# zhiqiangdon/pose-adv-aug

Measured on AMD Instinct MI355X. Metric: images/sec, 2-stack HG 256x256 bs=24 per GPU, full training step, higher is better.
Workload: dtype bf16; 1 GPU; BASELINE configs[1]: 2-stack hourglass chan 256, bs=24/GPU, 256x256 MPII-shape synthetic frames (720x1280 uint8 resident in HBM), on-device HumanAug warp, heat-map MSE, RMSprop, PCKh; global_batch=24, parallelism=dp1, ranks_seen=1, devices_seen=1

## Files before the change

pose_adv_aug_amd/csrc/api.hip:

```cpp
#include "../../include/poseadv.h"
#include "net.h"
#include "warp_bwd.h"
#include <stdio.h>
#include <string.h>
#include <new>
#include <string>

static thread_local char g_err[1024] = "";
void pa_set_error(const char* what, hipError_t e, const char* file, int line) {
    snprintf(g_err, sizeof g_err, "%s:%d: %s -> %s", file, line, what, hipGetErrorString(e));
}
void pa_set_error_msg(const char* msg) { snprintf(g_err, sizeof g_err, "%s", msg); }

struct pa_net { Net n; };
#define ST(s) reinterpret_cast<hipStream_t>(s)
#define TRY(x) do { int _r = (x); if (_r) { if (!g_err[0]) pa_set_error("kernel launch", (hipError_t)_r, __FILE__, __LINE__); return _r; } } while (0)
#define NEED_PTR(fn, p) do { if (!(p)) { pa_set_error_msg(fn ": " #p " is NULL"); return 1; } } while (0)
#define NEED_POS(fn, v) do { if ((v) < 1) { pa_set_error_msg(fn ": " #v " must be >= 1"); return 1; } } while (0)

extern "C" {

const char* pa_last_error(void) { return g_err; }
float pa_grad_scale(void) { return PA_GRAD_SCALE; }
int pa_dtype(void) { return PA_DTYPE_ID; }
// ... 321 lines not shown
    float* pbuf = nullptr; float* gbuf = nullptr;
    PA_CHECK(hipMallocAsync((void**)&pbuf, n.n_params * sizeof(float) * 2 + 64, n.st));
    gbuf = pbuf + ((n.n_params + 3) & ~(size_t)3);
    PA_CHECK(hipMemsetAsync(pbuf, 0, n.n_params * sizeof(float) * 2 + 64, n.st));
    PA_CHECK(hipMemcpyAsync(pbuf + op.c.p_w, w, (size_t)Cout * Cin * k * k * sizeof(float), hipMemcpyDeviceToDevice, n.st));
    if (bias) PA_CHECK(hipMemcpyAsync(pbuf + op.c.p_b, bias, Cout * sizeof(float), hipMemcpyDeviceToDevice, n.st));
    n.params = pbuf; n.grads = gbuf; n.buffers = pbuf;
    TRY(n.upload_tables());
    TRY(n.prepare_weights());
    n.train_bn = false;
    if (mode == 0) {
        TRY(pa_launch_nchw_f32_to_nhwc_bf16(a_in, op.xin, B, Cin, H, W, n.st));
        TRY(n.conv_fwd(op.c, pa_plain(op.xin), B, H, W, pa_none(), pa_none(), op.yout, nullptr));
        TRY(pa_launch_nhwc_bf16_to_nchw_f32(pa_plain(op.yout), out, B, Cout, H, W, n.st));
    } else if (mode == 1) {
        PaEpilogue ep; memset(&ep, 0, sizeof ep); ep.mode = PA_OUT_PLAIN;
        TRY(pa_launch_nchw_f32_to_nhwc_bf16(a_in, op.yout, B, Cout, H, W, n.st));
        TRY(n.conv_dgrad(op.c, pa_plain(op.yout), B, H, W, pa_none(), pa_none(), ep, op.xin));
        TRY(pa_launch_nhwc_bf16_to_nchw_f32(pa_plain(op.xin), out, B, Cin, H, W, n.st));
    } else {
        TRY(pa_launch_nchw_f32_to_nhwc_bf16(a_in, op.yout, B, Cout, H, W, n.st));
        TRY(pa_launch_nchw_f32_to_nhwc_bf16(b_in, op.xin, B, Cin, H, W, n.st));
        TRY(n.conv_wgrad(op.c, pa_plain(op.yout), pa_plain(op.xin), B, H, W));
        TRY(n.reduce_grads());
        PA_CHECK(hipMemcpyAsync(out, gbuf + op.c.p_w, (size_t)Cout * Cin * k * k * sizeof(float), hipMemcpyDeviceToDevice, n.st));
        if (out2) PA_CHECK(hipMemcpyAsync(out2, gbuf + op.c.p_b, Cout * sizeof(float), hipMemcpyDeviceToDevice, n.st));
    }
    PA_CHECK(hipStreamSynchronize(n.st));
    PA_CHECK(hipFree(pbuf));
    return 0;
}

struct WgradGroupOp {
    Net n; ConvLayer c[PA_WG_GROUP_MAX]; bf16 *dy[PA_WG_GROUP_MAX], *dyq[PA_WG_GROUP_MAX], *x[PA_WG_GROUP_MAX];
    float *pbuf = nullptr, *gbuf = nullptr;
    size_t build(const pa_wgrad_job* jobs, int nj, char* base) {
        Arena a; a.base = base;
        n.prep_jobs = a.get<PaPrepJob>(nj); n.red_jobs = a.get<PaWgradReduceJob>(nj); n.bneval_jobs = a.get<PaBnEvalJob>(1);
        for (int j = 0; j < nj; ++j) {
            const pa_wgrad_job& q = jobs[j];
            n.B = q.B;
            n.layout_conv(c[j], a, q.B * q.H * q.W, q.H, q.W);
            const size_t M = (size_t)q.B * q.H * q.W;
            dy[j] = a.get<bf16>(M * c[j].pcout);
            dyq[j] = q.dy_q ? a.get<bf16>(M * c[j].pcout) : nullptr;
            x[j] = a.get<bf16>(M * c[j].pcin);
        }
        pbuf = a.get<float>(n.n_params + 8);
        gbuf = a.get<float>(n.n_params + 8);
        a.take(0);
        return a.off;
    }
    int declare(const pa_wgrad_job* jobs, int nj) {
        if (nj < 1 || nj > PA_WG_GROUP_MAX) { pa_set_error_msg("pa_wgrad_group: 1 .. 8 jobs"); return 1; }
        n.is_agent = true;
        for (int j = 0; j < nj; ++j) {
            const pa_wgrad_job& q = jobs[j];
            if (q.Cin % 64 || q.Cout % 64 || (q.k != 1 && q.k != 3) || q.B < 1 || q.H < 1 || q.W < 1) { pa_set_error_msg("pa_wgrad_group: channels % 64 == 0, k in {1,3}"); return 1; }
            if ((q.dy_q == nullptr) != (q.dy_k == nullptr)) { pa_set_error_msg("pa_wgrad_group: dy_q and dy_k come together"); return 1; }
            char name[16]; snprintf(name, sizeof name, "j%d", j);
            n.declare_conv(c[j], name, q.Cin, q.Cout, q.k, q.db == nullptr);
        }
        return 0;
    }
};

size_t pa_wgrad_group_workspace_bytes(const pa_wgrad_job* jobs, int njobs) {
    g_err[0] = 0;
    WgradGroupOp op;
    if (op.declare(jobs, njobs)) return 0;
    return op.build(jobs, njobs, nullptr);
}

int pa_wgrad_group(const pa_wgrad_job* jobs, int njobs, int mode, void* ws, void* s) {
    g_err[0] = 0;
    WgradGroupOp op; Net& n = op.n;
    TRY(op.declare(jobs, njobs));
    n.st = ST(s);
    op.build(jobs, njobs, reinterpret_cast<char*>(ws));
    PA_CHECK(hipMemsetAsync(op.gbuf, 0, (n.n_params + 8) * sizeof(float), n.st));
    n.params = op.pbuf; n.grads = op.gbuf; n.buffers = op.pbuf;
    TRY(n.upload_tables());
    PaWgradArgs args[PA_WG_GROUP_MAX]; const PaWgradArgs* ptrs[PA_WG_GROUP_MAX];
    for (int j = 0; j < njobs; ++j) {
        const pa_wgrad_job& q = jobs[j];
        ConvLayer& c = op.c[j];
        TRY(pa_launch_nchw_f32_to_nhwc_bf16(q.dy, op.dy[j], q.B, q.Cout, q.H, q.W, n.st));
        if (q.dy_q) TRY(pa_launch_nchw_f32_to_nhwc_bf16(q.dy_q, op.dyq[j], q.B, q.Cout, q.H, q.W, n.st));
        TRY(pa_launch_nchw_f32_to_nhwc_bf16(q.x, op.x[j], q.B, q.Cin, q.H, q.W, n.st));
        PaWgradArgs& a = args[j]; memset(&a, 0, sizeof a);
        a.dy = pa_plain(op.dy[j]);
        if (q.dy_q) { a.dy.mode = PA_LD_LIN2; a.dy.q = op.dyq[j]; a.dy.k0 = q.dy_k; a.dy.k1 = q.dy_k + q.Cout; a.dy.k2 = q.dy_k + 2 * q.Cout; }
        a.x = pa_plain(op.x[j]);
        if (q.x_k) { a.x.mode = PA_LD_BNRELU; a.x.k0 = q.x_k; a.x.k1 = q.x_k + q.Cin; }
        a.part = c.part; a.dbpart = c.dbpart;
        a.B = q.B; a.H = q.H; a.W = q.W; a.Cin = c.pcin; a.Cout = c.pcout; a.taps = c.taps(); a.splits = c.splits;
        ptrs[j] = &a;
    }
    if (mode == 0) {
        for (int j = 0; j < njobs; ++j) TRY(pa_launch_wgrad(args[j], n.st));
    } else {
        for (int j = 0; j < njobs; ++j)
            if (pa_wgrad_job_workgroups(args[j]) == 0) { pa_set_error_msg("pa_wgrad_group: a job the grouped kernel does not take (shape / operand modes)"); return 2; }
        TRY(pa_launch_wgrad_group(ptrs, njobs, n.st, mode == 2));
    }
    TRY(pa_launch_wgrad_reduce(n.red_jobs, n.n_red, n.red_max, n.st));
    for (int j = 0; j < njobs; ++j) {
        const pa_wgrad_job& q = jobs[j];
        PA_CHECK(hipMemcpyAsync(q.dw, op.gbuf + op.c[j].p_w, (size_t)q.Cout * q.Cin * q.k * q.k * sizeof(float), hipMemcpyDeviceToDevice, n.st));
        if (q.db) PA_CHECK(hipMemcpyAsync(q.db, op.gbuf + op.c[j].p_b, q.Cout * sizeof(float), hipMemcpyDeviceToDevice, n.st));
    }
    PA_CHECK(hipStreamSynchronize(n.st));
    return 0;
}

int pa_conv2d_time(int mode, int variant, int B, int Cin, int Cout, int H, int W, int k, int iters, void* ws, float* ms_out, void* s) {
    g_err[0] = 0;
    ConvOp op; Net& n = op.n; n.is_agent = true; n.B = B; n.st = ST(s);
    n.declare_conv(op.c, "c", Cin, Cout, k, false);
    BNLayer bn_in, bn_out;
    n.declare_bn(bn_in, "bi", mode == 0 ? Cin : Cout);
    n.declare_bn(bn_out, "bo", mode == 0 ? Cout : Cin);
    Arena a; a.base = reinterpret_cast<char*>(ws);
    a.off = op.build(B, H, W, a.base);
    for (BNLayer* b : n.bns) n.layout_bn(*b, a, B * H * W);
    const size_t M = (size_t)B * H * W;
    bf16* extra = a.get<bf16>(M * (Cin > Cout ? Cin : Cout));
    bf16* extra2 = a.get<bf16>(M * (Cin > Cout ? Cin : Cout));
    float* pbuf = a.get<float>(2 * (n.n_params + 8));
    n.params = pbuf; n.grads = pbuf + n.n_params + 8; n.buffers = pbuf;
// ... 537 lines not shown
```

pose_adv_aug_amd/csrc/conv_wgrad.hip:

```cpp
#include "common.h"
#include "kernels.h"
#include "wgrad_reduce.h"
#include <stdlib.h>

template <int TN, int TK, int PMODE, int QMODE, int TAPS, bool STEM = false>
__global__ __launch_bounds__(256) void conv_wgrad_kernel(PaWgradArgs a) {
    constexpr int NI = TN / 32, KI = TK / 32;
    constexpr int MS = (TN + TK <= 128) ? 128 : 64;
    constexpr int MG = MS / 8;
    constexpr int NP = MG * TN / 8, NQ = MG * TK / 8;
    __shared__ __attribute__((aligned(16))) bf16 lds[(TN + TK) * MS];
    bf16* Pt = lds;
    bf16* Qt = lds + TN * MS;

    const int tid = threadIdx.x, lane = tid & 63, wave = tid >> 6;
    const int wn = wave & 1, wk = wave >> 1;
    const int M = a.B * a.H * a.W, HW = a.H * a.W;
    const int Kfull = TAPS * a.Cin;
    const int ktiles_per_tap = a.Cin / TK;
    const int split = blockIdx.x;
    const int tap = blockIdx.y / ktiles_per_tap;
    const int cbase = (blockIdx.y - tap * ktiles_per_tap) * TK;
    const int nbase = blockIdx.z * TN;
    const int dy = (TAPS == 9) ? tap / 3 - 1 : 0, dx = (TAPS == 9) ? tap - (tap / 3) * 3 - 1 : 0;
// ... 175 lines not shown
            float s = colsum[c];
            s += __shfl_xor(s, 1, 64); s += __shfl_xor(s, 2, 64); s += __shfl_xor(s, 4, 64);
            if (MG == 16) s += __shfl_xor(s, 8, 64);
            if (mg == 0) a.dbpart[(size_t)split * a.Cout + chan + c] = s;
        }
    }
}

template <int TN, int TK, int PMODE, int QMODE>
static void launch_w_taps(const PaWgradArgs& a, dim3 grid, hipStream_t st) {
    if (a.taps == 1) hipLaunchKernelGGL((conv_wgrad_kernel<TN, TK, PMODE, QMODE, 1>), grid, dim3(256), 0, st, a);
    else hipLaunchKernelGGL((conv_wgrad_kernel<TN, TK, PMODE, QMODE, 9>), grid, dim3(256), 0, st, a);
}

template <int TN, int TK>
static void launch_w_modes(const PaWgradArgs& a, dim3 grid, hipStream_t st) {
    const bool lin2 = a.dy.mode == PA_LD_LIN2, bnrelu = a.x.mode == PA_LD_BNRELU;
    if (lin2 && bnrelu) launch_w_taps<TN, TK, PA_LD_LIN2, PA_LD_BNRELU>(a, grid, st);
    else if (lin2) launch_w_taps<TN, TK, PA_LD_LIN2, PA_LD_PLAIN>(a, grid, st);
    else if (bnrelu) launch_w_taps<TN, TK, PA_LD_PLAIN, PA_LD_BNRELU>(a, grid, st);
    else launch_w_taps<TN, TK, PA_LD_PLAIN, PA_LD_PLAIN>(a, grid, st);
}

int pa_launch_stem_wgrad(const PaWgradArgs& a, hipStream_t st) {
    if (a.Cin != 256 || a.Cout != 64 || a.taps != 1 || a.x.mode != PA_LD_PLAIN || a.splits < 1) {
        pa_set_error_msg("pa_launch_stem_wgrad: bad arguments");
        return 1;
    }
    const PaWgradPlan p = pa_wgrad_launch_plan(a.B, a.H, a.W, a.Cin, a.Cout, a.taps, true, a.splits, false);
    if (p.path == PA_WGP_STEM_TILE) return pa_launch_stem_wgrad_tile(a, p, st);
    dim3 grid(a.splits, p.blocks, 1);
    if (a.dy.mode == PA_LD_LIN2)
        hipLaunchKernelGGL((conv_wgrad_kernel<64, 128, PA_LD_LIN2, PA_LD_PLAIN, 1, true>), grid, dim3(256), 0, st, a);
    else
        hipLaunchKernelGGL((conv_wgrad_kernel<64, 128, PA_LD_PLAIN, PA_LD_PLAIN, 1, true>), grid, dim3(256), 0, st, a);
    return (int)hipGetLastError();
}

int pa_launch_wgrad(const PaWgradArgs& a, hipStream_t st) {
    if ((a.taps != 1 && a.taps != 9) || a.Cin % 64 != 0 || a.Cout % 64 != 0 || a.splits < 1) {
        pa_set_error_msg("pa_launch_wgrad: channel counts must be multiples of 64, taps 1 or 9, splits >= 1");
        return 1;
    }
    const PaWgradPlan p = pa_wgrad_launch_plan(a.B, a.H, a.W, a.Cin, a.Cout, a.taps, false, a.splits, a.dbpart != nullptr);
    if (p.path == PA_WGP_TILE) return pa_launch_wgrad_tile(a, p, st);
    dim3 grid(a.splits, a.taps * a.Cin / p.cb, a.Cout / p.nb);
    if (p.nb == 128 && p.cb == 128) launch_w_modes<128, 128>(a, grid, st);
    else if (p.nb == 128) launch_w_modes<128, 64>(a, grid, st);
    else if (p.cb == 128) launch_w_modes<64, 128>(a, grid, st);
    else launch_w_modes<64, 64>(a, grid, st);
    return (int)hipGetLastError();
}

__global__ void wgrad_reduce_kernel(const PaWgradReduceJob* jobs) {
    wgrad_reduce_body(jobs[blockIdx.y], (int)blockIdx.x, (int)gridDim.x);
}

__global__ void wgrad_reduce_list_kernel(const PaWgradReduceJob* jobs, PaRedList list) {
    wgrad_reduce_body(jobs[list.idx[blockIdx.y]], (int)blockIdx.x, (int)gridDim.x);
}

int pa_launch_wgrad_reduce_list(const PaWgradReduceJob* jobs_dev, const int* idx, int n, int max_elems, hipStream_t st) {
    if (n <= 0) return 0;
    if (n > PA_RED_LIST_MAX) { pa_set_error_msg("pa_launch_wgrad_reduce_list: too many jobs"); return 1; }
    PaRedList list;
    for (int i = 0; i < PA_RED_LIST_MAX; ++i) list.idx[i] = idx[i < n ? i : 0];
    int bx = (max_elems + 255) / 256;
    if (bx > 576) bx = 576;
    if (bx < 1) bx = 1;
    hipLaunchKernelGGL(wgrad_reduce_list_kernel, dim3(bx, n), dim3(256), 0, st, jobs_dev, list);
    return (int)hipGetLastError();
}

int pa_launch_wgrad_reduce(const PaWgradReduceJob* jobs_dev, int njobs, int max_elems, hipStream_t st) {
    if (njobs <= 0) return 0;
    int bx = (max_elems + 255) / 256;
    if (bx > 576) bx = 576;
    if (bx < 1) bx = 1;
    hipLaunchKernelGGL(wgrad_reduce_kernel, dim3(bx, njobs), dim3(256), 0, st, jobs_dev);
    return (int)hipGetLastError();
}

__global__ __launch_bounds__(1024) void stem_wgrad_reduce_kernel(const float* part, int splits, float* dst, float* zero64) {
    __shared__ float red[4][256];
    const int n = blockIdx.x, k = threadIdx.x & 255, sl = threadIdx.x >> 8;
    if (zero64 && n == 0 && threadIdx.x < 64) zero64[threadIdx.x] = 0.f;
    const float* src = part + (size_t)n * 256 + k;
    float s = 0.f;
#pragma unroll 8
    for (int sp = sl; sp < splits; sp += 4) s += src[(size_t)sp * 64 * 256];
    red[sl][k] = s;
    __syncthreads();
    if (sl == 0) {
        const int ky = k >> 5, kx = (k & 31) >> 2, c = k & 3;
        if (ky < 7 && kx < 7 && c < 3) dst[((size_t)(n * 3 + c) * 7 + ky) * 7 + kx] = red[0][k] + red[1][k] + red[2][k] + red[3][k];
    }
}

int pa_launch_stem_wgrad_reduce(const float* part, int splits, float* dst, hipStream_t st, float* zero64) {
    hipLaunchKernelGGL(stem_wgrad_reduce_kernel, dim3(64), dim3(1024), 0, st, part, splits, dst, zero64);
    return (int)hipGetLastError();
}
```

pose_adv_aug_amd/csrc/conv_wgrad_tile.hip:

```cpp
#include "common.h"
#include "kernels.h"
#include "wgrad_reduce.h"
#include <stdlib.h>
#include <string.h>
#include <hip/hip_ext.h>

#ifndef PA_WG_NT
#define PA_WG_NT 0
#endif
#if PA_WG_NT
#define PA_WG_LOAD(p) __builtin_nontemporal_load(p)
#define PA_WG_STORE(p, v) __builtin_nontemporal_store(v, p)
#else
#define PA_WG_LOAD(p) (*(p))
#define PA_WG_STORE(p, v) (*(p) = (v))
#endif
#define PA_WG_RT 7
#define PA_WG_STEM 3
typedef short s16x4 __attribute__((ext_vector_type(4)));
typedef short s16x8 __attribute__((ext_vector_type(8)));

template <int CH>
__device__ __forceinline__ int wg_sw(int p) {
    return CH >= 128 ? ((p & 3) | ((p >> 1) & 4)) : (((p >> 1) & 1) | ((p >> 2) & 2));
}

template <int CH, class PixFn>
__device__ __forceinline__ bf16x8 wg_tr_frag(const bf16* tile, int gran, PixFn pix) {
    const int l = threadIdx.x & 63;
    s16x4 h[2];
#pragma unroll
    for (int hh = 0; hh < 2; ++hh) {
        const int p = pix(8 * (l >> 4) + 4 * hh + ((l & 15) >> 2));
        const bf16* ptr = tile + p * CH + ((gran ^ wg_sw<CH>(p)) << 4) + 4 * (l & 3);
        h[hh] = __builtin_amdgcn_ds_read_tr16_b64_v4i16((__attribute__((address_space(3))) s16x4*)(ptr));
    }
    s16x8 v = __builtin_shufflevector(h[0], h[1], 0, 1, 2, 3, 4, 5, 6, 7);
    return __builtin_bit_cast(bf16x8, v);
}

__device__ __forceinline__ void wg_lds_barrier() { asm volatile("s_waitcnt lgkmcnt(0)\n\ts_barrier" ::: "memory"); }

template <int TAPS, int NF, int CF, int WNW>
constexpr int wg_lds_elems() { return 128 * (16 * NF * WNW) + (TAPS == 9 ? 10 * 32 : 128) * (16 * CF * (4 / WNW)); }

template <int TAPS, int NF, int CF, int WNW, int PMODE, int QMODE, bool DB, bool PIPE>
__device__ __forceinline__ void wgrad_tile_body(const PaWgradArgs& a, int ntiles, int split, int S, int by, int bz, bf16* lds) {
    constexpr int WCW = 4 / WNW;
    constexpr int NB = 16 * NF * WNW, CB = 16 * CF * WCW;
    constexpr int PW = 18, PWL = 32, HP = TAPS == 9 ? 180 : 128, HPL = TAPS == 9 ? 10 * PWL : 128;
    constexpr int CPN = NB / 8, CPC = CB / 8;
    constexpr int PASS_N = 128 * CPN / 256;
    constexpr int PASS_C = (HP * CPC + 255) / 256;
    static_assert(128 * NB + HPL * CB == wg_lds_elems<TAPS, NF, CF, WNW>(), "LDS size");
    bf16* dyT = lds;
    bf16* xT = lds + 128 * NB;

    const int tid = threadIdx.x, lane = tid & 63;
    const int wave = __builtin_amdgcn_readfirstlane(tid >> 6);
    const int wn = wave % WNW, wc = wave / WNW;
    const int n0 = by * NB, c0 = bz * CB;
    const int M = a.B * a.H * a.W;
    const int tiles_x = TAPS == 9 ? a.W / 16 : 1, tiles_y = TAPS == 9 ? a.H / 8 : 1;
    const int Kfull = TAPS * a.Cin;

    const int nchunk = tid % CPN, cchunk = tid % CPC;
    const bool want_db = DB && a.dbpart != nullptr && bz == 0;
    const bool p_lin2 = PMODE == PA_LD_LIN2 || (PMODE == PA_WG_RT && a.dy.mode == PA_LD_LIN2);
    const bool q_bnrelu = QMODE == PA_LD_BNRELU || (QMODE == PA_WG_RT && a.x.mode == PA_LD_BNRELU);
    static_assert(!PIPE || (PMODE != PA_WG_RT && QMODE != PA_WG_RT), "run-time modes: plain form only");
    float colsum[8];
#pragma unroll
    for (int j = 0; j < 8; ++j) colsum[j] = 0.f;

    f32x4 acc[TAPS][CF][NF];
#pragma unroll
    for (int t = 0; t < TAPS; ++t)
#pragma unroll
        for (int cf = 0; cf < CF; ++cf)
#pragma unroll
            for (int f = 0; f < NF; ++f) acc[t][cf][f] = f32x4{0.f, 0.f, 0.f, 0.f};

    auto mfma_tile = [&]() {
        if (TAPS == 9) {
            int doff[NF][2], xoff[3][2];
#pragma unroll
            for (int hh = 0; hh < 2; ++hh) {
                const int kl = 8 * (lane >> 4) + 4 * hh + ((lane & 15) >> 2);
#pragma unroll
                for (int f = 0; f < NF; ++f) doff[f][hh] = kl * NB + (((wn * NF + f) ^ wg_sw<NB>(kl)) << 4) + 4 * (lane & 3);
#pragma unroll
                for (int d = 0; d < 3; ++d) {
                    const int col = (kl & 15) + d;
                    xoff[d][hh] = ((kl >> 4) * PWL + col) * CB + ((wc ^ wg_sw<CB>(col)) << 4) + 4 * (lane & 3);
                }
            }
            auto tr8 = [&](const bf16* base, int o0, int o1) {
                s16x4 h0 = __builtin_amdgcn_ds_read_tr16_b64_v4i16((__attribute__((address_space(3))) s16x4*)(base + o0));
                s16x4 h1 = __builtin_amdgcn_ds_read_tr16_b64_v4i16((__attribute__((address_space(3))) s16x4*)(base + o1));
                s16x8 v = __builtin_shufflevector(h0, h1, 0, 1, 2, 3, 4, 5, 6, 7);
// ... 165 lines not shown
            __builtin_amdgcn_sched_barrier(0);
            wg_lds_barrier();
            mfma_tile();
        }
    } else
    for (int tile = split; tile < ntiles; tile += S) {
        int b = 0, y0 = 0, x0 = 0;
        if (TAPS == 9) {
            int t = tile;
            x0 = (t % tiles_x) * 16; t /= tiles_x;
            y0 = (t % tiles_y) * 8;
            b = t / tiles_y;
        }
        if (tile != split) __syncthreads();
        {
            bf16x8 rp[PASS_N], rq[PASS_N];
            bool ok[PASS_N];
            float pk0[8], pk1[8], pk2[8];
            if (p_lin2) {
#pragma unroll
                for (int j = 0; j < 8; ++j) {
                    pk0[j] = a.dy.k0[n0 + nchunk * 8 + j]; pk1[j] = a.dy.k1[n0 + nchunk * 8 + j]; pk2[j] = a.dy.k2[n0 + nchunk * 8 + j];
                }
            }
            constexpr int UNP = TAPS == 9 ? 2 : PASS_N;
#pragma unroll
            for (int u0 = 0; u0 < PASS_N; u0 += UNP) {
#pragma unroll
                for (int v = 0; v < UNP; ++v) {
                    const int u = u0 + v;
                    const int r = u * (256 / CPN) + tid / CPN;
                    int m;
                    if (TAPS == 9) { m = (b * a.H + y0 + (r >> 4)) * a.W + x0 + (r & 15); ok[u] = true; }
                    else { m = tile * 128 + r; ok[u] = m < M; }
                    const size_t idx = ok[u] ? (size_t)m * a.Cout + n0 + nchunk * 8 : 0;
                    rp[u] = PA_WG_LOAD(reinterpret_cast<const bf16x8*>(a.dy.p + idx));
                    if (p_lin2) rq[u] = PA_WG_LOAD(reinterpret_cast<const bf16x8*>(a.dy.q + idx));
                }
#pragma unroll
                for (int v = 0; v < UNP; ++v) {
                    const int u = u0 + v;
                    const int r = u * (256 / CPN) + tid / CPN;
                    bf16x8 o;
                    if (p_lin2) {
#pragma unroll
                        for (int j = 0; j < 8; ++j) o[j] = (bf16)fmaf(pk0[j], (float)rp[u][j], fmaf(pk1[j], (float)rq[u][j], pk2[j]));
                    } else {
                        o = rp[u];
                    }
                    if (!ok[u]) {
#pragma unroll
                        for (int j = 0; j < 8; ++j) o[j] = (bf16)0.f;
                    }
                    if (DB && want_db) {
#pragma unroll
                        for (int j = 0; j < 8; ++j) colsum[j] += (float)o[j];
                    }
                    *reinterpret_cast<bf16x8*>(dyT + r * NB + (((nchunk >> 1) ^ wg_sw<NB>(r)) << 4) + (nchunk & 1) * 8) = o;
                }
            }
        }
        {
            bf16x8 rx[PASS_C];
            bool ok[PASS_C];
            float qk0[8], qk1[8];
            if (q_bnrelu) {
#pragma unroll
                for (int j = 0; j < 8; ++j) { qk0[j] = a.x.k0[c0 + cchunk * 8 + j]; qk1[j] = a.x.k1[c0 + cchunk * 8 + j]; }
            }
            int sb = 0, sy = 0, sx = 0;
            if (QMODE == PA_WG_STEM) {
                const int m0 = tile * 128 + tid / CPC, HWo = a.H * a.W;
                sb = m0 / HWo; const int rem = m0 - sb * HWo; sy = rem / a.W; sx = rem - sy * a.W;
            }
#pragma unroll
            for (int u = 0; u < PASS_C; ++u) {
                const int hp = u * (256 / CPC) + tid / CPC;
                int m;
                if (TAPS == 9) {
                    const int hy = hp / PW, hx = hp - hy * PW;
                    const int y = y0 + hy - 1, x = x0 + hx - 1;
                    ok[u] = hp < HP && (unsigned)y < (unsigned)a.H && (unsigned)x < (unsigned)a.W;
                    m = (b * a.H + y) * a.W + x;
                } else { m = tile * 128 + hp; ok[u] = m < M; }
                if (QMODE == PA_WG_STEM) {
                    const int chunk = c0 / 8 + cchunk, ky = chunk >> 2, q = chunk & 3;
                    const int Hin = 2 * a.H, Win = 2 * a.W;
                    const int bb = ok[u] ? sb : 0, y = ok[u] ? sy : 0, x = ok[u] ? sx : 0;
                    sx += 256 / CPC;
                    while (sx >= a.W) { sx -= a.W; if (++sy >= a.H) { sy = 0; ++sb; } }
                    const int yi = 2 * y + ky - 3, xi = 2 * x + 2 * q - 3;
                    const bool rowok = ok[u] && ky < 7 && (unsigned)yi < (unsigned)Hin;
                    const bool lok = rowok && (unsigned)xi < (unsigned)Win, hok = rowok && (unsigned)(xi + 1) < (unsigned)Win;
                    const bf16* rowp = a.x.p + ((size_t)bb * Hin + (rowok ? yi : 0)) * Win * 4;
                    bf16x4 lo = *reinterpret_cast<const bf16x4*>(rowp + (size_t)(lok ? xi : 0) * 4);
                    bf16x4 hi = *reinterpret_cast<const bf16x4*>(rowp + (size_t)(hok ? xi + 1 : 0) * 4);
                    const bf16x4 z = {(bf16)0.f, (bf16)0.f, (bf16)0.f, (bf16)0.f};
                    if (!lok) lo = z;
                    if (!hok) hi = z;
                    rx[u] = __builtin_shufflevector(lo, hi, 0, 1, 2, 3, 4, 5, 6, 7);
                    ok[u] = true;
                    continue;
                }
                const size_t idx = ok[u] ? (size_t)m * a.Cin + c0 + cchunk * 8 : 0;
                rx[u] = PA_WG_LOAD(reinterpret_cast<const bf16x8*>(a.x.p + idx));
            }
#pragma unroll
            for (int u = 0; u < PASS_C; ++u) {
                const int hi = u * (256 / CPC) + tid / CPC;
                const int hp = TAPS == 9 ? (hi / PW) * PWL + hi % PW : hi;
                if (hi < HP) {
                    bf16x8 o;
                    if (q_bnrelu) {
#pragma unroll
                        for (int j = 0; j < 8; ++j) o[j] = (bf16)fmaxf(fmaf(qk0[j], (float)rx[u][j], qk1[j]), 0.f);
                    } else {
                        o = rx[u];
                    }
                    if (!ok[u]) {
#pragma unroll
                        for (int j = 0; j < 8; ++j) o[j] = (bf16)0.f;
                    }
                    *reinterpret_cast<bf16x8*>(xT + hp * CB + (((cchunk >> 1) ^ wg_sw<CB>(hp)) << 4) + (cchunk & 1) * 8) = o;
                }
            }
        }
        __syncthreads();
        mfma_tile();
    }

    float* slab = a.part + (size_t)split * a.Cout * Kfull;
#pragma unroll
    for (int f = 0; f < NF; ++f) {
        const int n = n0 + (wn * NF + f) * 16 + (lane & 15);
#pragma unroll
        for (int t = 0; t < TAPS; ++t)
#pragma unroll
            for (int cf = 0; cf < CF; ++cf) {
                const int c = c0 + (wc * CF + cf) * 16 + (lane >> 4) * 4;
                PA_WG_STORE(reinterpret_cast<f32x4*>(slab + (size_t)n * Kfull + t * a.Cin + c), acc[t][cf][f]);
            }
    }
    if (DB && want_db) {
        __syncthreads();
        float* red = reinterpret_cast<float*>(lds);
#pragma unroll
        for (int j = 0; j < 8; ++j) red[tid * 8 + j] = colsum[j];
        __syncthreads();
        if (tid < NB) {
            const int ch = tid >> 3, j = tid & 7;
            float s = 0.f;
            for (int r = ch; r < 256; r += CPN) s += red[r * 8 + j];
            a.dbpart[(size_t)split * a.Cout + n0 + tid] = s;
        }
    }
}

template <int TAPS, int NF, int CF, int WNW, int PMODE, int QMODE, bool DB, bool PIPE = false, int OCC = 1>
__global__ __launch_bounds__(256, PIPE ? OCC : 2) void wgrad_tile_kernel(PaWgradArgs a, int ntiles) {
    __shared__ __attribute__((aligned(16))) bf16 lds[wg_lds_elems<TAPS, NF, CF, WNW>()];
    wgrad_tile_body<TAPS, NF, CF, WNW, PMODE, QMODE, DB, PIPE>(a, ntiles, (int)blockIdx.x, (int)gridDim.x, (int)blockIdx.y, (int)blockIdx.z, lds);
}

#define PA_WG_MAXJOBS 8
struct PaWgradGroup {
    PaWgradArgs a[PA_WG_MAXJOBS];
    int ntiles[PA_WG_MAXJOBS], S[PA_WG_MAXJOBS], ny[PA_WG_MAXJOBS], kind[PA_WG_MAXJOBS];
    int begin[PA_WG_MAXJOBS + 1];
    int njobs;
    const PaWgradReduceJob* red_jobs;
    PaRedList red;
    int red_n, red_wgs;
};

__global__ __launch_bounds__(256, 2) void wgrad_group_kernel(PaWgradGroup g) {
    constexpr int L9 = wg_lds_elems<9, 4, 1, 1>(), L1 = wg_lds_elems<1, 4, 4, 2>();
    __shared__ __attribute__((aligned(16))) bf16 lds[L9 > L1 ? L9 : L1];
    const int id = (int)blockIdx.x;
    if (id >= g.begin[g.njobs]) {
        const int local = id - g.begin[g.njobs];
        for (int i = 0; i < g.red_n; ++i) wgrad_reduce_body(g.red_jobs[g.red.idx[i]], local, g.red_wgs);
        return;
    }
    int j = 0;
#pragma unroll
    for (int k = 1; k < PA_WG_MAXJOBS; ++k) if (k < g.njobs && id >= g.begin[k]) j = k;
    const int local = id - g.begin[j];
    const int S = g.S[j], split = local % S, rest = local / S, by = rest % g.ny[j], bz = rest / g.ny[j];
    const PaWgradArgs& a = g.a[j];
    const int nt = g.ntiles[j];
    switch (g.kind[j]) {
        case PA_WGK_9_44: wgrad_tile_body<9, 4, 1, 1, PA_LD_PLAIN, PA_LD_BNRELU, false, false>(a, nt, split, S, by, bz, lds); break;
        case PA_WGK_9_44L: wgrad_tile_body<9, 4, 1, 1, PA_LD_LIN2, PA_LD_BNRELU, false, false>(a, nt, split, S, by, bz, lds); break;
        case PA_WGK_1_44: wgrad_tile_body<1, 4, 4, 2, PA_WG_RT, PA_WG_RT, true, false>(a, nt, split, S, by, bz, lds); break;
        case PA_WGK_1_42: wgrad_tile_body<1, 4, 2, 2, PA_WG_RT, PA_WG_RT, true, false>(a, nt, split, S, by, bz, lds); break;
        case PA_WGK_1_24: wgrad_tile_body<1, 2, 4, 2, PA_WG_RT, PA_WG_RT, true, false>(a, nt, split, S, by, bz, lds); break;
        default: wgrad_tile_body<1, 2, 2, 2, PA_WG_RT, PA_WG_RT, true, false>(a, nt, split, S, by, bz, lds); break;
    }
}

static thread_local unsigned g_wt_launch_flags = 0;
void pa_wgrad_set_launch_flags(unsigned flags) { g_wt_launch_flags = flags; }

template <int TAPS, int NF, int CF, int WNW, bool PIPE>
static void launch_wt_modes2(const PaWgradArgs& a, dim3 grid, int ntiles, hipStream_t st) {
    const bool lin2 = a.dy.mode == PA_LD_LIN2, bnrelu = a.x.mode == PA_LD_BNRELU;
    constexpr bool DB = TAPS == 1;
    const unsigned fl = g_wt_launch_flags;
    auto go = [&](auto kernel) {
        if (fl) hipExtLaunchKernelGGL(kernel, grid, dim3(256), 0, st, nullptr, nullptr, fl, a, ntiles);
        else hipLaunchKernelGGL(kernel, grid, dim3(256), 0, st, a, ntiles);
    };
    if (lin2 && bnrelu) go(wgrad_tile_kernel<TAPS, NF, CF, WNW, PA_LD_LIN2, PA_LD_BNRELU, DB, PIPE>);
    else if (lin2) go(wgrad_tile_kernel<TAPS, NF, CF, WNW, PA_LD_LIN2, PA_LD_PLAIN, DB, PIPE>);
    else if (bnrelu) go(wgrad_tile_kernel<TAPS, NF, CF, WNW, PA_LD_PLAIN, PA_LD_BNRELU, DB, PIPE>);
    else go(wgrad_tile_kernel<TAPS, NF, CF, WNW, PA_LD_PLAIN, PA_LD_PLAIN, DB, PIPE>);
}

template <int TAPS, int NF, int CF, int WNW>
static void launch_wt_modes(const PaWgradArgs& a, dim3 grid, int ntiles, hipStream_t st) {
    if (!pa_tuning().wgrad_nopipe && ntiles >= 2 * (int)grid.x) launch_wt_modes2<TAPS, NF, CF, WNW, true>(a, grid, ntiles, st);
    else launch_wt_modes2<TAPS, NF, CF, WNW, false>(a, grid, ntiles, st);
}

int pa_launch_stem_wgrad_tile(const PaWgradArgs& a, const PaWgradPlan& p, hipStream_t st) {
    dim3 grid(a.splits, 1, 1);
    if (a.dy.mode == PA_LD_LIN2) hipLaunchKernelGGL((wgrad_tile_kernel<1, 2, 8, 2, PA_LD_LIN2, PA_WG_STEM, false>), grid, dim3(256), 0, st, a, p.ntiles);
    else hipLaunchKernelGGL((wgrad_tile_kernel<1, 2, 8, 2, PA_LD_PLAIN, PA_WG_STEM, false>), grid, dim3(256), 0, st, a, p.ntiles);
    return (int)hipGetLastError();
}

int pa_launch_wgrad_tile(const PaWgradArgs& a, const PaWgradPlan& p, hipStream_t st) {
    dim3 grid(a.splits, a.Cout / p.nb, a.Cin / p.cb);
    if (a.taps == 9) launch_wt_modes<9, 4, 1, 1>(a, grid, p.ntiles, st);
    else if (p.nb == 128 && p.cb == 128) launch_wt_modes<1, 4, 4, 2>(a, grid, p.ntiles, st);
    else if (p.nb == 128) launch_wt_modes<1, 4, 2, 2>(a, grid, p.ntiles, st);
    else if (p.cb == 128) launch_wt_modes<1, 2, 4, 2>(a, grid, p.ntiles, st);
    else launch_wt_modes<1, 2, 2, 2>(a, grid, p.ntiles, st);
    return (int)hipGetLastError();
}

static bool wg_job_plan(const PaWgradArgs& a, PaWgradPlan& p) {
    p = pa_wgrad_launch_plan(a.B, a.H, a.W, a.Cin, a.Cout, a.taps, false, a.splits, a.dbpart != nullptr);
    if (p.group_kind < 0) return false;
    if (a.dy.mode != PA_LD_PLAIN && a.dy.mode != PA_LD_LIN2) return false;
    if (a.x.mode != PA_LD_PLAIN && a.x.mode != PA_LD_BNRELU) return false;
    return a.taps != 9 || a.x.mode == PA_LD_BNRELU;
}

int pa_wgrad_job_workgroups(const PaWgradArgs& a) {
    PaWgradPlan p;
    return wg_job_plan(a, p) ? a.splits * p.blocks : 0;
}

int pa_launch_wgrad_group(const PaWgradArgs* const* as, int n, hipStream_t st, bool keep_order, const PaWgradReduceJob* red_jobs, const int* red_idx, int red_n) {
    if (n < 1 || n > PA_WG_MAXJOBS) { pa_set_error_msg("pa_launch_wgrad_group: 1 .. 8 jobs"); return 1; }
    if (red_n < 0 || red_n > PA_RED_LIST_MAX || (red_n > 0 && (!red_jobs || !red_idx))) { pa_set_error_msg("pa_launch_wgrad_group: bad reduction list"); return 1; }
    PaWgradGroup g;
    memset(&g, 0, sizeof g);
    int order[PA_WG_MAXJOBS]; long work[PA_WG_MAXJOBS];
    PaWgradPlan ps[PA_WG_MAXJOBS];
    for (int j = 0; j < n; ++j) {
        if (!wg_job_plan(*as[j], ps[j])) { pa_set_error_msg("pa_launch_wgrad_group: a job the grouped kernel does not take"); return 1; }
        order[j] = j;
        work[j] = (long)((ps[j].ntiles + as[j]->splits - 1) / as[j]->splits) * (as[j]->taps == 9 ? 3 : 2);
    }
    for (int i = 1; i < n && !keep_order; ++i)
        for (int k = i; k > 0 && work[order[k]] > work[order[k - 1]]; --k) { const int t = order[k]; order[k] = order[k - 1]; order[k - 1] = t; }
    int begin = 0;
    for (int jj = 0; jj < n; ++jj) {
        const int j = order[jj];
        const PaWgradPlan& p = ps[j];
        g.a[jj] = *as[j]; g.ntiles[jj] = p.ntiles; g.S[jj] = as[j]->splits; g.ny[jj] = as[j]->Cout / p.nb;
        g.kind[jj] = p.group_kind == PA_WGK_9_44 && as[j]->dy.mode == PA_LD_LIN2 ? PA_WGK_9_44L : p.group_kind;
        g.begin[jj] = begin;
        begin += as[j]->splits * p.blocks;
    }
    g.begin[n] = begin; g.njobs = n;
    if (red_n > 0) {
        const int rw = pa_tuning().wg_red_wgs < 1 ? 1 : pa_tuning().wg_red_wgs;
        g.red_jobs = red_jobs; g.red_n = red_n; g.red_wgs = rw;
        for (int i = 0; i < PA_RED_LIST_MAX; ++i) g.red.idx[i] = red_idx[i < red_n ? i : 0];
        begin += rw;
    }
    hipLaunchKernelGGL(wgrad_group_kernel, dim3(begin), dim3(256), 0, st, g);
    return (int)hipGetLastError();
}
```

pose_adv_aug_amd/csrc/tuning.h:

```cpp
#pragma once
#include <stdlib.h>

#define PA_TUNING_TABLE(X)                                                                                                           \
                                                                      \
    X(conv1_old,        "PA_CONV1_OLD",        0,   "1x1 convolutions on the generic kernel (no row-tile kernel, no fused upsample-add gradient)") \
    X(conv3_old,        "PA_CONV3_OLD",        0,   "3x3 convolutions on the generic kernel (no halo-tile kernel)")                 \
    X(wgrad_old,        "PA_WGRAD_OLD",        0,   "weight gradients on the generic kernel (no tile kernel, stem included)")       \
    X(stem_wgrad_old,   "PA_STEM_WGRAD_OLD",   0,   "the stem's weight gradient on the generic kernel")                            \
    X(eltwise_old,      "PA_ELTWISE_OLD",      0,   "pooling / upsample-add / cell-mask launches in their first, unvectorised form") \
    X(conv3_nosmall,    "PA_CONV3_NOSMALL",    0,   "no 8 x 8 / 4 x 4 halo tiles: the small maps go to the generic kernel")        \
    X(igemm_oneshot,    "PA_IGEMM_ONESHOT",    1,   "0: the small 1x1 layers on the K-stepping generic kernel instead of the one-shot one") \
    X(no_dz3,           "PA_NO_DZ3",           0,   "conv3's data gradient does not store dz3 (its readers recompute it)")         \
    X(no_dz2,           "PA_NO_DZ2",           0,   "conv2's data gradient does not store dz2")                                    \
    X(epi_bwd_direct,   "PA_EPI_BWD_DIRECT",   0,   "direct (no LDS) BatchNorm-backward epilogue wherever an instance carries both") \
    X(conv3_noxcd,      "PA_CONV3_NOXCD",      0,   "3x3 tiles in launch order instead of one contiguous range per XCD")           \
    X(wg_group,         "PA_WG_GROUP",         1,   "0: one launch per weight gradient instead of group launches")                 \
    X(wg_red_in_group,  "PA_WG_RED_IN_GROUP",  1,   "0: slab reductions as launches of their own instead of inside the next group launch") \
    X(wgrad_anyorder,   "PA_WGRAD_ANYORDER",   1,   "0: ungrouped weight gradients of one flush as ordinary in-order launches")    \
    X(wgrad_nopipe,     "PA_WGRAD_NOPIPE",     0,   "plain instead of pipelined tile weight gradients")                            \
    X(upadd_fuse,       "PA_UPADD_FUSE",       1,   "0: the upsample-add backward's low-resolution half as a launch of its own")   \
    X(upadd_split,      "PA_UPADD_SPLIT",      1,   "0: both halves of the upsample-add backward in one launch on the main stream") \
    X(pool_route,       "PA_POOL_ROUTE",       3,   "pool gradients through the forward pools' arg-max maps: bit 0 the hourglass pools, bit 1 the stem's pool (0: a pool backward launch each)") \
    X(fin_prologue,     "PA_FIN_PROLOGUE",     128, "most partial rows a consumer finalizes in its prologue (0: always a finalize launch; at most 128)") \
    X(fin_mask,         "PA_FIN_MASK",         7,   "which finalizes may ride in a consumer: 1 forward x1 / x2, 2 backward x2, 4 backward x3") \
    X(single_stream,    "PA_SINGLE_STREAM",    0,   "everything on the caller's stream")                                           \
    X(no_wstream,       "PA_NO_WSTREAM",       0,   "side streams, but the weight gradients on the stream that produced their operands") \
    X(stem_on_main,     "PA_STEM_ON_MAIN",     1,   "0: the stem's weight gradient on the weight-gradient stream")                 \
                                                              \
    X(wgrad_wgs1,       "PA_WGRAD_WGS1",       256, "workgroup target of a 1x1 tile weight gradient launched alone")               \
    X(wgrad_wgs9,       "PA_WGRAD_WGS9",       256, "the same for 3x3")                                                            \
    X(wgrad_min1,       "PA_WGRAD_MIN1",       3,   "fewest 128-pixel tiles for which a 1x1 weight gradient takes the tile kernel") \
    X(wg_group_wgs1,    "PA_WG_GROUP_WGS1",    64,  "workgroup budget of a 1x1 job of a group launch")                             \
    X(wg_group_wgs9,    "PA_WG_GROUP_WGS9",    64,  "the same for 3x3")                                                            \
    X(wg_group_minper1, "PA_WG_GROUP_MINPER1", 2,   "fewest tiles per workgroup of a 1x1 job")                                     \
    X(wg_group_minper9, "PA_WG_GROUP_MINPER9", 4,   "the same for 3x3")                                                            \
    X(wg_group_cap,     "PA_WG_GROUP_CAP",     256, "most workgroups of one group launch")                                         \
    X(wg_red_wgs,       "PA_WG_RED_WGS",       256, "workgroups of the slab reduction inside a group launch")                      \
    X(wreduce_lag,      "PA_WREDUCE_LAG",      2,   "flushes whose slabs wait in the stash before they are summed")                \
    X(stem_splits,      "PA_STEM_SPLITS",      512, "splits (slabs) of the stem's weight gradient")                                \
    X(wgrad_tile1,      "PA_WGRAD_TILE1",      0,   "generic 1x1 weight gradient: forced tile variant (0: by shape)")              \
    X(wgrad_tile9,      "PA_WGRAD_TILE9",      0,   "the same for 3x3")                                                            \
    X(wgrad_blocks,     "PA_WGRAD_BLOCKS",     0,   "generic weight gradient: forced split count (0: by shape)")                   \
                                                                                    \
    X(ablate,           "PA_ABLATE",           0,   "INSTRUMENT, wrong results: mask of launch classes that are skipped (net.hip)") \
    X(ablate_h,         "PA_ABLATE_H",         8,   "INSTRUMENT: largest map height the low-resolution bits of PA_ABLATE skip")    \
    X(conv3_dbg,        "PA_CONV3_DBG",        0,   "INSTRUMENT, wrong results: phase ablation / tap rotation / cycle stamps of the 3x3 tile kernel") \
    X(conv1_dbg,        "PA_CONV1_DBG",        0,   "INSTRUMENT, timing only: cycle stamps of the one-shot 1x1 kernel")            \
    X(conv1t_dbg,       "PA_CONV1T_DBG",       0,   "INSTRUMENT, timing only: cycle stamps of the row-tile 1x1 kernel")            \
    X(fin_anyorder,     "PA_FIN_ANYORDER",     0,   "INSTRUMENT, results may be wrong: finalize launches without ordering behind their producer")

struct PaTuning {
#define PA_TUNING_FIELD(field, env, value, doc) int field = value;
    PA_TUNING_TABLE(PA_TUNING_FIELD)
#undef PA_TUNING_FIELD
};

#ifdef PA_TUNING
inline const PaTuning& pa_tuning() {
    static const PaTuning t = [] {
        PaTuning v;
#define PA_TUNING_READ(field, env, value, doc) if (const char* e = getenv(env)) v.field = atoi(e);
        PA_TUNING_TABLE(PA_TUNING_READ)
#undef PA_TUNING_READ
        return v;
    }();
    return t;
}
#else
inline const PaTuning& pa_tuning() {
    static constexpr PaTuning t{};
    return t;
}
#endif
```

pose_adv_aug_amd/csrc/wgrad_plan.h:

```cpp
#pragma once
#include "tuning.h"

enum PaWgradPath {
    PA_WGP_GENERIC,
    PA_WGP_TILE,
    PA_WGP_STEM_TILE,
    PA_WGP_STEM_GENERIC
};
enum { PA_WGK_9_44 = 0, PA_WGK_9_44L, PA_WGK_1_44, PA_WGK_1_42, PA_WGK_1_24, PA_WGK_1_22, PA_WGK_N };

struct PaWgradPlan {
    int path;
    int nb, cb;
    int ntiles;
    int splits;
    int group_splits;
    int group_kind;
    int blocks;
};

inline int pa_wgrad_balanced(int ntiles, int s) {
    const int per = (ntiles + s - 1) / s;
    return (ntiles + per - 1) / per;
}

inline PaWgradPlan pa_wgrad_generic_plan(int M, int Cin, int Cout, int taps, bool stem) {
    const PaTuning& t = pa_tuning();
    PaWgradPlan p{};
    p.path = stem ? PA_WGP_STEM_GENERIC : PA_WGP_GENERIC; p.group_kind = -1;
    const int f = taps == 1 ? t.wgrad_tile1 : t.wgrad_tile9;
    p.nb = Cout % 128 == 0 && f != 1 && f != 3 ? 128 : 64;
    p.cb = Cin % 128 == 0 && f != 1 && f != 2 ? 128 : 64;
    p.blocks = (Cout / p.nb) * (taps * Cin / p.cb);
    const int ms = p.nb + p.cb <= 128 ? 128 : 64;
    p.ntiles = (M + ms - 1) / ms;
    const int target = t.wgrad_blocks >= 8 ? t.wgrad_blocks : (taps == 9 ? 1024 : 512);
    const int s = ((target + p.blocks - 1) / p.blocks + 7) & ~7;
    p.splits = s > p.ntiles ? (p.ntiles < 1 ? 1 : p.ntiles) : s;
    if (stem) { p.nb = 64; p.cb = 128; p.ntiles = (M + 63) / 64; p.blocks = 2; }
    return p;
}

inline PaWgradPlan pa_wgrad_plan(int B, int H, int W, int Cin, int Cout, int taps, bool stem) {
    const PaTuning& t = pa_tuning();
    const bool shaped = H > 0 && W > 0;
    const int M = shaped ? B * H * W : B;
    PaWgradPlan p = pa_wgrad_generic_plan(M, Cin, Cout, taps, stem);
    if (stem) {
        const int ntiles = (M + 127) / 128;
        if (t.stem_splits > 0 && t.stem_splits <= ntiles) p.splits = t.stem_splits;
        if (!t.wgrad_old && !t.stem_wgrad_old) { p.path = PA_WGP_STEM_TILE; p.nb = 64; p.cb = 256; p.ntiles = ntiles; p.blocks = 1; }
        return p;
    }
    if (t.wgrad_old || !shaped || Cin % 64 || Cout % 64 || (taps != 1 && taps != 9)) return p;
    const int nb = taps == 1 && Cout % 128 == 0 ? 128 : 64, cb = taps == 1 && Cin % 128 == 0 ? 128 : 64;
    const int ntiles = taps == 9 ? B * (H / 8) * (W / 16) : (M + 127) / 128;
    if (taps == 9 && (H % 8 || W % 16 || ntiles < 48)) return p;
    if (taps == 1 && ntiles < t.wgrad_min1) return p;
    p.path = PA_WGP_TILE; p.nb = nb; p.cb = cb; p.ntiles = ntiles; p.blocks = (Cout / nb) * (Cin / cb);
    int s = (taps == 9 ? t.wgrad_wgs9 : t.wgrad_wgs1) / p.blocks;
    p.splits = pa_wgrad_balanced(ntiles, s < 1 ? 1 : s > ntiles ? ntiles : s);
    if (!t.wg_group) return p;
    s = (taps == 9 ? t.wg_group_wgs9 : t.wg_group_wgs1) / p.blocks;
    const int minper = taps == 9 ? t.wg_group_minper9 : t.wg_group_minper1;
    if (s * minper > ntiles) s = ntiles / minper;
    p.group_splits = pa_wgrad_balanced(ntiles, s < 1 ? 1 : s);
    p.group_kind = taps == 9 ? PA_WGK_9_44 : nb == 128 ? (cb == 128 ? PA_WGK_1_44 : PA_WGK_1_42) : (cb == 128 ? PA_WGK_1_24 : PA_WGK_1_22);
    return p;
}

inline int pa_wgrad_layer_splits(const PaWgradPlan& p, bool as_job) { return as_job && p.group_splits > 0 ? p.group_splits : p.splits; }

inline PaWgradPlan pa_wgrad_launch_plan(int B, int H, int W, int Cin, int Cout, int taps, bool stem, int splits, bool bias_grad) {
    const PaWgradPlan p = pa_wgrad_plan(B, H, W, Cin, Cout, taps, stem);
    const bool refused = splits < 1 || splits > p.ntiles || (taps == 9 && bias_grad);
    return (p.path == PA_WGP_TILE || p.path == PA_WGP_STEM_TILE) && refused ? pa_wgrad_generic_plan(B * H * W, Cin, Cout, taps, stem) : p;
}
```

Before: 4243 images/sec.

## Shrink group wgrad tiles to raise occupancy to three workgroups per CU

The grouped weight-gradient kernel now uses smaller per-workgroup tiles (64 output channels; 32 input channels for 3x3, 64/128 for 1x1) and launch bounds of three workgroups per CU, with LDS capped to fit. The split count stays fixed by the old block budget, so there are more workgroups, and the workgroup cap is raised to match. When a 1x1 layer's nominal tile is 128 wide, its bias-gradient column sums are computed in a separate pass over the staged dy tile. The aim is better latency hiding and fuller CU occupancy, at the cost of less reuse per tile and extra LDS reads.

```diff
diff --git a/pose_adv_aug_amd/csrc/api.hip b/pose_adv_aug_amd/csrc/api.hip
--- a/pose_adv_aug_amd/csrc/api.hip
+++ b/pose_adv_aug_amd/csrc/api.hip
@@ -397,7 +397,7 @@
         return a.off;
     }
     int declare(const pa_wgrad_job* jobs, int nj) {
-        if (nj < 1 || nj > PA_WG_GROUP_MAX) { pa_set_error_msg("pa_wgrad_group: 1 .. 8 jobs"); return 1; }
+        if (!jobs || nj < 1 || nj > PA_WG_GROUP_MAX) { pa_set_error_msg("pa_wgrad_group: 1 .. 8 jobs"); return 1; }
         n.is_agent = true;
         for (int j = 0; j < nj; ++j) {
             const pa_wgrad_job& q = jobs[j];
@@ -421,6 +421,9 @@
     g_err[0] = 0;
     WgradGroupOp op; Net& n = op.n;
     TRY(op.declare(jobs, njobs));
+    if (!ws) { pa_set_error_msg("pa_wgrad_group: ws is null"); return 1; }
+    for (int j = 0; j < njobs; ++j)
+        if (!jobs[j].dy || !jobs[j].x || !jobs[j].dw) { pa_set_error_msg("pa_wgrad_group: dy, x and dw of every job must be set"); return 1; }
     n.st = ST(s);
     op.build(jobs, njobs, reinterpret_cast<char*>(ws));
     PA_CHECK(hipMemsetAsync(op.gbuf, 0, (n.n_params + 8) * sizeof(float), n.st));
diff --git a/pose_adv_aug_amd/csrc/conv_wgrad.hip b/pose_adv_aug_amd/csrc/conv_wgrad.hip
--- a/pose_adv_aug_amd/csrc/conv_wgrad.hip
+++ b/pose_adv_aug_amd/csrc/conv_wgrad.hip
@@ -251,11 +251,11 @@
     return (int)hipGetLastError();
 }
 
-__global__ void wgrad_reduce_kernel(const PaWgradReduceJob* jobs) {
+__global__ __launch_bounds__(256) void wgrad_reduce_kernel(const PaWgradReduceJob* jobs) {
     wgrad_reduce_body(jobs[blockIdx.y], (int)blockIdx.x, (int)gridDim.x);
 }
 
-__global__ void wgrad_reduce_list_kernel(const PaWgradReduceJob* jobs, PaRedList list) {
+__global__ __launch_bounds__(256) void wgrad_reduce_list_kernel(const PaWgradReduceJob* jobs, PaRedList list) {
     wgrad_reduce_body(jobs[list.idx[blockIdx.y]], (int)blockIdx.x, (int)gridDim.x);
 }
 
diff --git a/pose_adv_aug_amd/csrc/conv_wgrad_tile.hip b/pose_adv_aug_amd/csrc/conv_wgrad_tile.hip
--- a/pose_adv_aug_amd/csrc/conv_wgrad_tile.hip
+++ b/pose_adv_aug_amd/csrc/conv_wgrad_tile.hip
@@ -22,7 +22,8 @@
 
 template <int CH>
 __device__ __forceinline__ int wg_sw(int p) {
-    return CH >= 128 ? ((p & 3) | ((p >> 1) & 4)) : (((p >> 1) & 1) | ((p >> 2) & 2));
+    static_assert(CH == 32 || CH == 64 || CH >= 128, "granule swizzle: 2, 4 or >= 8 granules per pixel row");
+    return CH >= 128 ? ((p & 3) | ((p >> 1) & 4)) : CH == 64 ? (((p >> 1) & 1) | ((p >> 2) & 2)) : ((p >> 3) & 1);
 }
 
 template <int CH, class PixFn>
@@ -45,7 +46,7 @@
 constexpr int wg_lds_elems() { return 128 * (16 * NF * WNW) + (TAPS == 9 ? 10 * 32 : 128) * (16 * CF * (4 / WNW)); }
 
 template <int TAPS, int NF, int CF, int WNW, int PMODE, int QMODE, bool DB, bool PIPE>
-__device__ __forceinline__ void wgrad_tile_body(const PaWgradArgs& a, int ntiles, int split, int S, int by, int bz, bf16* lds) {
+__device__ __forceinline__ void wgrad_tile_body(const PaWgradArgs& a, int ntiles, int split, int S, int by, int bz, bf16* lds, bool db16 = false) {
     constexpr int WCW = 4 / WNW;
     constexpr int NB = 16 * NF * WNW, CB = 16 * CF * WCW;
     constexpr int PW = 18, PWL = 32, HP = TAPS == 9 ? 180 : 128, HPL = TAPS == 9 ? 10 * PWL : 128;
@@ -317,7 +318,7 @@
 #pragma unroll
                         for (int j = 0; j < 8; ++j) o[j] = (bf16)0.f;
                     }
-                    if (DB && want_db) {
+                    if (DB && want_db && !db16) {
 #pragma unroll
                         for (int j = 0; j < 8; ++j) colsum[j] += (float)o[j];
                     }
@@ -391,6 +392,16 @@
             }
         }
         __syncthreads();
+        if (DB && want_db && db16 && tid < 128) {
+            const int ch = tid & 7, rg = tid >> 3;
+#pragma unroll 1
+            for (int u = 0; u < 8; ++u) {
+                const int r = u * 16 + rg;
+                const bf16x8 o = *reinterpret_cast<const bf16x8*>(dyT + r * NB + (((ch >> 1) ^ wg_sw<NB>(r)) << 4) + (ch & 1) * 8);
+#pragma unroll
+                for (int j = 0; j < 8; ++j) colsum[j] += (float)o[j];
+            }
+        }
         mfma_tile();
     }
 
@@ -415,7 +426,7 @@
         if (tid < NB) {
             const int ch = tid >> 3, j = tid & 7;
             float s = 0.f;
-            for (int r = ch; r < 256; r += CPN) s += red[r * 8 + j];
+            for (int r = ch; r < (db16 ? 128 : 256); r += CPN) s += red[r * 8 + j];
             a.dbpart[(size_t)split * a.Cout + n0 + tid] = s;
         }
     }
@@ -431,6 +442,7 @@
 struct PaWgradGroup {
     PaWgradArgs a[PA_WG_MAXJOBS];
     int ntiles[PA_WG_MAXJOBS], S[PA_WG_MAXJOBS], ny[PA_WG_MAXJOBS], kind[PA_WG_MAXJOBS];
+    int db16[PA_WG_MAXJOBS];
     int begin[PA_WG_MAXJOBS + 1];
     int njobs;
     const PaWgradReduceJob* red_jobs;
@@ -438,9 +450,11 @@
     int red_n, red_wgs;
 };
 
-__global__ __launch_bounds__(256, 2) void wgrad_group_kernel(PaWgradGroup g) {
-    constexpr int L9 = wg_lds_elems<9, 4, 1, 1>(), L1 = wg_lds_elems<1, 4, 4, 2>();
+__global__ __launch_bounds__(256, 3) void wgrad_group_kernel(PaWgradGroup g) {
+    constexpr int L9 = wg_lds_elems<9, 2, 1, 2>(), L14 = wg_lds_elems<1, 2, 4, 2>(), L12 = wg_lds_elems<1, 2, 2, 2>();
+    constexpr int L1 = L14 > L12 ? L14 : L12;
     __shared__ __attribute__((aligned(16))) bf16 lds[L9 > L1 ? L9 : L1];
+    static_assert(sizeof(lds) <= 53248, "a group workgroup takes no more LDS than a three-per-CU workgroup of the main chain");
     const int id = (int)blockIdx.x;
     if (id >= g.begin[g.njobs]) {
         const int local = id - g.begin[g.njobs];
@@ -454,13 +468,12 @@
     const int S = g.S[j], split = local % S, rest = local / S, by = rest % g.ny[j], bz = rest / g.ny[j];
     const PaWgradArgs& a = g.a[j];
     const int nt = g.ntiles[j];
+    const bool db16 = g.db16[j] != 0;
     switch (g.kind[j]) {
-        case PA_WGK_9_44: wgrad_tile_body<9, 4, 1, 1, PA_LD_PLAIN, PA_LD_BNRELU, false, false>(a, nt, split, S, by, bz, lds); break;
-        case PA_WGK_9_44L: wgrad_tile_body<9, 4, 1, 1, PA_LD_LIN2, PA_LD_BNRELU, false, false>(a, nt, split, S, by, bz, lds); break;
-        case PA_WGK_1_44: wgrad_tile_body<1, 4, 4, 2, PA_WG_RT, PA_WG_RT, true, false>(a, nt, split, S, by, bz, lds); break;
-        case PA_WGK_1_42: wgrad_tile_body<1, 4, 2, 2, PA_WG_RT, PA_WG_RT, true, false>(a, nt, split, S, by, bz, lds); break;
-        case PA_WGK_1_24: wgrad_tile_body<1, 2, 4, 2, PA_WG_RT, PA_WG_RT, true, false>(a, nt, split, S, by, bz, lds); break;
-        default: wgrad_tile_body<1, 2, 2, 2, PA_WG_RT, PA_WG_RT, true, false>(a, nt, split, S, by, bz, lds); break;
+        case PA_WGK_9_21: wgrad_tile_body<9, 2, 1, 2, PA_LD_PLAIN, PA_LD_BNRELU, false, false>(a, nt, split, S, by, bz, lds); break;
+        case PA_WGK_9_21L: wgrad_tile_body<9, 2, 1, 2, PA_LD_LIN2, PA_LD_BNRELU, false, false>(a, nt, split, S, by, bz, lds); break;
+        case PA_WGK_1_24: wgrad_tile_body<1, 2, 4, 2, PA_WG_RT, PA_WG_RT, true, false>(a, nt, split, S, by, bz, lds, db16); break;
+        default: wgrad_tile_body<1, 2, 2, 2, PA_WG_RT, PA_WG_RT, true, false>(a, nt, split, S, by, bz, lds, db16); break;
     }
 }
 
@@ -515,7 +528,7 @@
 
 int pa_wgrad_job_workgroups(const PaWgradArgs& a) {
     PaWgradPlan p;
-    return wg_job_plan(a, p) ? a.splits * p.blocks : 0;
+    return wg_job_plan(a, p) ? a.splits * p.group_blocks : 0;
 }
 
 int pa_launch_wgrad_group(const PaWgradArgs* const* as, int n, hipStream_t st, bool keep_order, const PaWgradReduceJob* red_jobs, const int* red_idx, int red_n) {
@@ -536,10 +549,11 @@
     for (int jj = 0; jj < n; ++jj) {
         const int j = order[jj];
         const PaWgradPlan& p = ps[j];
-        g.a[jj] = *as[j]; g.ntiles[jj] = p.ntiles; g.S[jj] = as[j]->splits; g.ny[jj] = as[j]->Cout / p.nb;
-        g.kind[jj] = p.group_kind == PA_WGK_9_44 && as[j]->dy.mode == PA_LD_LIN2 ? PA_WGK_9_44L : p.group_kind;
+        g.a[jj] = *as[j]; g.ntiles[jj] = p.ntiles; g.S[jj] = as[j]->splits; g.ny[jj] = as[j]->Cout / p.group_nb;
+        g.kind[jj] = p.group_kind == PA_WGK_9_21 && as[j]->dy.mode == PA_LD_LIN2 ? PA_WGK_9_21L : p.group_kind;
+        g.db16[jj] = as[j]->taps == 1 && p.nb == 128;
         g.begin[jj] = begin;
-        begin += as[j]->splits * p.blocks;
+        begin += as[j]->splits * p.group_blocks;
     }
     g.begin[n] = begin; g.njobs = n;
     if (red_n > 0) {
diff --git a/pose_adv_aug_amd/csrc/tuning.h b/pose_adv_aug_amd/csrc/tuning.h
--- a/pose_adv_aug_amd/csrc/tuning.h
+++ b/pose_adv_aug_amd/csrc/tuning.h
@@ -30,11 +30,11 @@
     X(wgrad_wgs1,       "PA_WGRAD_WGS1",       256, "workgroup target of a 1x1 tile weight gradient launched alone")               \
     X(wgrad_wgs9,       "PA_WGRAD_WGS9",       256, "the same for 3x3")                                                            \
     X(wgrad_min1,       "PA_WGRAD_MIN1",       3,   "fewest 128-pixel tiles for which a 1x1 weight gradient takes the tile kernel") \
-    X(wg_group_wgs1,    "PA_WG_GROUP_WGS1",    64,  "workgroup budget of a 1x1 job of a group launch")                             \
+    X(wg_group_wgs1,    "PA_WG_GROUP_WGS1",    64,  "budget of nb x cb blocks of a 1x1 job of a group launch (fixes its split count)") \
     X(wg_group_wgs9,    "PA_WG_GROUP_WGS9",    64,  "the same for 3x3")                                                            \
     X(wg_group_minper1, "PA_WG_GROUP_MINPER1", 2,   "fewest tiles per workgroup of a 1x1 job")                                     \
     X(wg_group_minper9, "PA_WG_GROUP_MINPER9", 4,   "the same for 3x3")                                                            \
-    X(wg_group_cap,     "PA_WG_GROUP_CAP",     256, "most workgroups of one group launch")                                         \
+    X(wg_group_cap,     "PA_WG_GROUP_CAP",     512, "most tile workgroups of one group launch (the reduction's ride on top)")      \
     X(wg_red_wgs,       "PA_WG_RED_WGS",       256, "workgroups of the slab reduction inside a group launch")                      \
     X(wreduce_lag,      "PA_WREDUCE_LAG",      2,   "flushes whose slabs wait in the stash before they are summed")                \
     X(stem_splits,      "PA_STEM_SPLITS",      512, "splits (slabs) of the stem's weight gradient")                                \
diff --git a/pose_adv_aug_amd/csrc/wgrad_plan.h b/pose_adv_aug_amd/csrc/wgrad_plan.h
--- a/pose_adv_aug_amd/csrc/wgrad_plan.h
+++ b/pose_adv_aug_amd/csrc/wgrad_plan.h
@@ -7,7 +7,7 @@
     PA_WGP_STEM_TILE,
     PA_WGP_STEM_GENERIC
 };
-enum { PA_WGK_9_44 = 0, PA_WGK_9_44L, PA_WGK_1_44, PA_WGK_1_42, PA_WGK_1_24, PA_WGK_1_22, PA_WGK_N };
+enum { PA_WGK_9_21 = 0, PA_WGK_9_21L, PA_WGK_1_24, PA_WGK_1_22, PA_WGK_N };
 
 struct PaWgradPlan {
     int path;
@@ -17,6 +17,8 @@
     int group_splits;
     int group_kind;
     int blocks;
+    int group_nb, group_cb;
+    int group_blocks;
 };
 
 inline int pa_wgrad_balanced(int ntiles, int s) {
@@ -65,7 +67,9 @@
     const int minper = taps == 9 ? t.wg_group_minper9 : t.wg_group_minper1;
     if (s * minper > ntiles) s = ntiles / minper;
     p.group_splits = pa_wgrad_balanced(ntiles, s < 1 ? 1 : s);
-    p.group_kind = taps == 9 ? PA_WGK_9_44 : nb == 128 ? (cb == 128 ? PA_WGK_1_44 : PA_WGK_1_42) : (cb == 128 ? PA_WGK_1_24 : PA_WGK_1_22);
+    p.group_nb = 64; p.group_cb = taps == 9 ? 32 : cb;
+    p.group_blocks = (Cout / p.group_nb) * (Cin / p.group_cb);
+    p.group_kind = taps == 9 ? PA_WGK_9_21 : cb == 128 ? PA_WGK_1_24 : PA_WGK_1_22;
     return p;
 }
 
```

Result: no change. 4255 images/sec (median of 5 runs) (+0.3%).
